# GregoryFaust/yaha

Hardware: AMD Instinct MI355X
Metric: aligned reads/s (whole node), 1 000 bp reads, OQC mode hot path (higher is better)
Workload: dtype int16

## Files before the change

### include/yaha_hip.h

```cpp
#ifndef YAHA_HIP_H
#define YAHA_HIP_H
#include <stdint.h>
#include <stddef.h>
#ifdef __cplusplus
extern "C" {
#endif

#define YGPU_OK            0
#define YGPU_EINVAL      (-1)
#define YGPU_ENODEV      (-2)
#define YGPU_ENOMEM      (-3)
#define YGPU_EOVERFLOW   (-4)
#define YGPU_EINTERNAL   (-5)
#define YGPU_EBUSY       (-6)

typedef struct ygpu_params {
    int32_t wordLen;
    int32_t maxHits;
    int32_t bandWidth;
    int32_t maxGap;
    int32_t maxIntron;
    int32_t minMatch;
    int32_t maxDesert;
    int32_t minNonOverlap;
// ... 181 lines not shown
int  ygpu_junctions_collect(ygpu_ctx *ctx, ygpu_junction *out, uint64_t stats[4]);

int  ygpu_inject_results(ygpu_ctx *ctx, const ygpu_result_batch *r);
int  ygpu_selftest_primitives(ygpu_ctx *ctx, uint32_t n, uint32_t seed, int key_bits);
int  ygpu_trace_volume(ygpu_ctx *ctx, uint64_t out[6]);

typedef uint64_t ygpu_ticket;
int  ygpu_submit(ygpu_ctx *ctx, const ygpu_read_batch *batch, ygpu_ticket *ticket);
int  ygpu_poll(ygpu_ctx *ctx, ygpu_ticket ticket);
int  ygpu_wait(ygpu_ctx *ctx, ygpu_ticket ticket, ygpu_result_batch *out);
int  ygpu_last_timing(ygpu_ctx *ctx, float *total_ms, int *n_stages, const char *const **names, const float **ms);


typedef struct ygpu_fragment {
    uint32_t startRefOff;
    uint16_t startQueryOff, endQueryOff;
    uint16_t refLen;
    uint16_t reserved;
    uint32_t read_strand;
} ygpu_fragment;

int  ygpu_seed_join(ygpu_ctx *ctx, const ygpu_fragment **frags, uint64_t *n_frags);

int  ygpu_chain(ygpu_ctx *ctx, const ygpu_fragment **clump_frags, const uint32_t **clump_frag_start,
                const uint32_t **clump_read_strand, uint64_t *n_clumps);

enum { YGPU_DP_FULL = 0, YGPU_DP_BANDED = 1, YGPU_DP_EXT_FWD = 2, YGPU_DP_EXT_REV = 3 };
typedef struct ygpu_dp_problem {
    uint32_t read;
    uint8_t  strand;
    uint8_t  mode;
    uint16_t qOff;
    uint16_t qLen;
    uint16_t rLen;
    uint32_t rOff;
} ygpu_dp_problem;
typedef struct ygpu_dp_result {
    int32_t  score;
    uint16_t addedQLen, addedRLen;
    uint32_t op_start, n_ops;
} ygpu_dp_result;
int  ygpu_dp_batch(ygpu_ctx *ctx, const ygpu_dp_problem *problems, uint32_t n,
                   const ygpu_dp_result **results, const uint32_t **ops, uint64_t *n_ops);
enum { YGPU_DP_KERNELS_AUTO = 0, YGPU_DP_KERNELS_WAVE = 1, YGPU_DP_KERNELS_LANES = 2, YGPU_DP_KERNELS_LANES_CAREFUL = 3 };
int  ygpu_dp_batch_ex(ygpu_ctx *ctx, const ygpu_dp_problem *problems, uint32_t n, int kernels,
                      const ygpu_dp_result **results, const uint32_t **ops, uint64_t *n_ops);
// ... 50 lines not shown
```

### yaha_amd/__init__.py

```python
import ctypes as C
import os

_HERE = os.path.dirname(os.path.abspath(__file__))
LIB_PATH = os.environ.get("YAHA_HIP_LIB", os.path.join(_HERE, "csrc", "libyaha_hip.so"))
CLI_PATH = os.path.join(_HERE, "csrc", "yaha")


class Params(C.Structure):
    _fields_ = [(n, C.c_int32) for n in (
        "wordLen", "maxHits", "bandWidth", "maxGap", "maxIntron", "minMatch", "maxDesert", "minNonOverlap",
        "minRawScore", "minExtLength", "GOCost", "GECost", "RCost", "MScore", "XCutoff")] + [("minIdentity", C.c_float)]


class IndexView(C.Structure):
    _fields_ = [("bases", C.c_void_p), ("n_base_bytes", C.c_uint64), ("maxROff", C.c_uint32),
                ("startingOffs", C.c_void_p), ("ROA", C.c_void_p), ("totalMatches", C.c_uint32), ("wordLen", C.c_int32)]


class ReadBatch(C.Structure):
    _fields_ = [("n_reads", C.c_uint32), ("codes", C.c_void_p), ("offsets", C.c_void_p)]


class Clump(C.Structure):
    _fields_ = [("sro", C.c_uint32), ("sqo", C.c_uint16), ("eqo", C.c_uint16), ("refLen", C.c_uint16),
# ... 131 lines not shown
    _fields_ = [("n_reads", C.c_uint32), ("clump_start", C.POINTER(C.c_uint32)), ("clumps", C.POINTER(OutClump)), ("ops", C.POINTER(C.c_uint32)),
                ("n_clumps", C.c_uint64), ("n_ops", C.c_uint64), ("counters", Counters)]


class ArenaProfile(C.Structure):
    _fields_ = [("n", C.c_uint32), ("last_clump_slots", C.c_uint32), ("cap", C.c_uint64 * 224), ("trace_ratio", C.c_double), ("ops_ratio", C.c_double), ("last_fall", C.c_int64), ("bases", C.c_uint64)]


DP_FULL, DP_BANDED, DP_EXT_FWD, DP_EXT_REV = 0, 1, 2, 3
DP_KERNELS_AUTO, DP_KERNELS_WAVE, DP_KERNELS_LANES, DP_KERNELS_LANES_CAREFUL = 0, 1, 2, 3

EXPORTS = (
    "ygpu_device_count", "ygpu_init", "ygpu_init_multi", "ygpu_clone", "ygpu_destroy", "ygpu_last_error", "ygpu_memory", "ygpu_park", "ygpu_get_arena_profile", "ygpu_presize", "ygpu_upload", "ygpu_upload_nowait", "ygpu_run", "ygpu_collect", "ygpu_result_size", "ygpu_collect_into", "ygpu_host_alloc", "ygpu_host_free", "ygpu_set_postfilter", "ygpu_postfilter_snapshot", "ygpu_postfilter", "ygpu_postfilter_drop", "ygpu_inject_results", "ygpu_selftest_primitives", "ygpu_trace_volume", "ygpu_filtered_size", "ygpu_collect_filtered", "ygpu_last_timing",
    "ygpu_depth_enable", "ygpu_depth_size", "ygpu_depth_collect", "yaha_session_depth_params",
    "ygpu_events_enable", "ygpu_events_size", "ygpu_events_collect", "yaha_session_events_params",
    "ygpu_pileup_enable", "ygpu_pileup_size", "ygpu_pileup_collect", "ygpu_pileup_candidates_size", "ygpu_pileup_candidates_collect", "ygpu_pileup_gather",
    "yaha_session_pileup_params",
    "ygpu_pileup_add", "ygpu_snv_call_size", "ygpu_snv_collect", "yaha_session_snv_params",
    "ygpu_indels_enable", "ygpu_indels_size", "ygpu_indels_collect", "yaha_session_indel_params",
    "ygpu_eprofile_enable", "ygpu_eprofile_size", "ygpu_eprofile_collect", "yaha_session_eprofile_params",
    "ygpu_junctions_enable", "ygpu_junctions_size", "ygpu_junctions_collect", "yaha_session_junction_params",
    "ygpu_bgzf_open", "ygpu_bgzf_bound", "ygpu_bgzf_compress", "ygpu_bgzf_last_error", "ygpu_bgzf_close",
    "ygpu_bamsort_open", "ygpu_bamsort_append", "ygpu_bamsort_sort", "ygpu_bamsort_next", "ygpu_bamsort_info", "ygpu_bamsort_last_error", "ygpu_bamsort_close",
    "ygpu_submit", "ygpu_poll", "ygpu_wait", "ygpu_seed_join", "ygpu_chain", "ygpu_dp_batch", "ygpu_dp_batch_ex",
    "yaha_session_open", "yaha_session_close", "yaha_session_error", "yaha_session_params",
    "yaha_session_index_view", "yaha_session_header", "yaha_session_next_batch", "yaha_session_emit", "yaha_session_postfilter_params", "yaha_session_emit_filtered",
    "yaha_build_index", "yaha_main")

_lib = None


def lib():
    global _lib
    if _lib is None:
        if not os.path.exists(LIB_PATH):
            raise RuntimeError("%s is missing: run `python -c 'import __graft_entry__ as g; g.build()'` "
                               "(or make -C yaha_amd/csrc); there is no fallback path" % LIB_PATH)
        L = C.CDLL(LIB_PATH)
        L.ygpu_last_error.restype = C.c_char_p
        L.yaha_session_error.restype = C.c_char_p
        L.ygpu_bgzf_last_error.restype = C.c_char_p
        L.ygpu_bgzf_last_error.argtypes = [C.c_void_p]
        L.ygpu_bgzf_bound.restype = C.c_uint64
        L.ygpu_bgzf_bound.argtypes = [C.c_uint64]
        L.ygpu_bamsort_last_error.restype = C.c_char_p
        L.ygpu_bamsort_last_error.argtypes = [C.c_void_p]
        L.ygpu_bamsort_info.restype = C.c_uint64
# ... 264 lines not shown
        nc, no = C.c_uint64(), C.c_uint64()
        self._check(lib().ygpu_filtered_size(self._h, C.byref(nc), C.byref(no)), "ygpu_filtered_size")
        self._f_cs = (C.c_uint32 * (n_reads + 1))(); self._f_cl = (OutClump * max(1, nc.value))(); self._f_ops = (C.c_uint32 * max(1, no.value))()
        r = FilteredBatch()
        self._check(lib().ygpu_collect_filtered(self._h, self._f_cs, self._f_cl, self._f_ops, C.byref(r)), "ygpu_collect_filtered")
        return r

    def trace_volume(self):
        v = (C.c_uint64 * 6)()
        self._check(lib().ygpu_trace_volume(self._h, v), "ygpu_trace_volume")
        return {"records_written": v[0], "records_visitable": v[1], "calls": v[2], "walkers": v[3], "record_bytes": v[4], "arena_bytes": v[5]}

    def timing(self):
        tot, n = C.c_float(), C.c_int()
        names, ms = C.POINTER(C.c_char_p)(), C.POINTER(C.c_float)()
        self._check(lib().ygpu_last_timing(self._h, C.byref(tot), C.byref(n), C.byref(names), C.byref(ms)), "ygpu_last_timing")
        return tot.value, {names[i].decode(): ms[i] for i in range(n.value)}

    def seed_join(self):
        f, n = C.POINTER(Fragment)(), C.c_uint64()
        self._check(lib().ygpu_seed_join(self._h, C.byref(f), C.byref(n)), "ygpu_seed_join")
        return f, n.value

    def chain(self):
        f, s, rs, n = C.POINTER(Fragment)(), C.POINTER(C.c_uint32)(), C.POINTER(C.c_uint32)(), C.c_uint64()
        self._check(lib().ygpu_chain(self._h, C.byref(f), C.byref(s), C.byref(rs), C.byref(n)), "ygpu_chain")
        return f, s, rs, n.value

    def dp_batch(self, problems, kernels=DP_KERNELS_AUTO):
        arr = (DPProblem * len(problems))(*problems)
        res, ops, nops = C.POINTER(DPResult)(), C.POINTER(C.c_uint32)(), C.c_uint64()
        self._check(lib().ygpu_dp_batch_ex(self._h, arr, len(problems), kernels, C.byref(res), C.byref(ops), C.byref(nops)), "ygpu_dp_batch_ex")
        return res, ops, nops.value

    def submit(self, batch):
        t = C.c_uint64()
        self._check(lib().ygpu_submit(self._h, C.byref(batch), C.byref(t)), "ygpu_submit")
        return t.value

    def poll(self, ticket):
        return lib().ygpu_poll(self._h, C.c_uint64(ticket))

    def wait(self, ticket):
        r = ResultBatch()
        self._check(lib().ygpu_wait(self._h, C.c_uint64(ticket), C.byref(r)), "ygpu_wait")
        return r
# ... 136 lines not shown
```

### yaha_amd/csrc/device/ctx.h

```cpp
#pragma once
#include <hip/hip_runtime.h>
#include <string>
#include <vector>
#include <cstring>
#include <cstdio>
#include <cstdlib>
#include <algorithm>
#include <array>
#include <atomic>
#include <chrono>
#include <thread>
#include <mutex>
#include <condition_variable>
#include <memory>
#include "common.h"
#include "../oqc_core.h"

#define HIPCHK(call) do { hipError_t e_ = (call); \
    if (e_ != hipSuccess) { ctx->err = std::string(#call) + ": " + hipGetErrorString(e_); return YGPU_ENODEV; } } while (0)

#define KL(kern, grid, block, shmem, st, ...) do { hipLaunchKernelGGL(kern, grid, block, shmem, st, __VA_ARGS__); hipError_t e_ = hipGetLastError(); \
    if (e_ != hipSuccess) { ctx->err = std::string("launch of " #kern " failed: ") + hipGetErrorString(e_); return YGPU_ENODEV; } } while (0)

#define YD_MAX_CHUNK_EV 16
// ... 9 lines not shown
        if (keep && p && cap) { hipMemcpyAsync(np, p, cap, hipMemcpyDeviceToDevice, st); hipStreamSynchronize(st); }
        if (p) hipFree(p);
        p = np; cap = ncap; return 0;
    }
    void release() { if (p) hipFree(p); p = nullptr; cap = 0; }
    int ensureExact(size_t bytes)
    {
        if (bytes <= cap) return 0;
        release();
        void *np = nullptr;
        if (hipMalloc(&np, bytes) != hipSuccess) return -1;
        p = np; cap = bytes; return 0;
    }
    template <class T> T *as() const { return (T *)p; }
};

enum {
    CNT_NMULTI = 0, CNT_MAXN, CNT_CLUMPS, CNT_CFRAGS, CNT_QCHAIN, CNT_QALIGN, CNT_OUTCLUMPS, CNT_OUTOPS, CNT_QDP, CNT_DPOPS, CNT_NBIG, CNT_QBIG,
    CNT_STATEOPS, CNT_EXTOPS, CNT_QEXT, CNT_SLOW, CNT_NDP, CNT_NDP16, CNT_GAPOPS, CNT_NPEND,
    CNT_NMULTI2 ,
        CNT_NTINY, CNT_NSMALL, CNT_NMID, CNT_NB12, CNT_NB16,
        CNT_NB24,
    CNT_SEGC,
    CNT_NFRAGS = CNT_SEGC + 16,
    CNT_NREG = CNT_NFRAGS + 3,
    CNT_SCANFAIL = CNT_NREG + 2,
    CNT_N = CNT_NREG + 4
};
enum { T_SEED = 0, T_SORT, T_FRAGS, T_CHAIN, T_ALIGN, T_LAYOUT, T_TOP, T_P1 = T_TOP, T_XROWS, T_XTRACE, T_P3, T_XROWS_DEV, T_XROWS_PK, T_N };

extern std::atomic<int> gCtxPerDevice[64];
extern std::mutex gRowsMu[64];
extern hipEvent_t gRowsEv[64][4];
extern bool gRowsEvValid[64][4];
extern unsigned long long gRowsSeq[64];
extern std::atomic<int> gActiveRuns[64];
extern const char *const kStageNames[T_N];

struct PfSide {
    std::string err;
    hipStream_t stream = nullptr;
    uint32_t *pinned = nullptr;
    hipEvent_t evSync = nullptr;
    DevBuf scanState, counters;
    int device = 0;
};

// ... 70 lines not shown
    DevCounters *snapCtr = nullptr;
    DevCounters snapCtrPlain{};
    unsigned long long snapHits = 0, snapFrags = 0, snapRegions = 0;
    DevBuf oqCs, oqCl, oqOpsIn, oqSeeds, oqQlen;
    std::shared_ptr<TrackImage> track[TRACK_KINDS];
    DevBuf puFwd, puReadOff, puTileCnt, puTileStart, puCand, puSlots, puRows;
    uint64_t puNCand = 0; bool puHaveCand = false;
    DevBuf snvOut;
    uint64_t snvN = 0; bool snvHave = false;
    DevBuf idTable, idStats, idSeqStart, idSeqLen, idBinBase, idTileCnt, idTileStart, idOut;
    bool idSet = false, idAuto = false;
    uint64_t idCap = 0, snapBases = 0;
    uint32_t idMinMapq = 0, idMinLen = 1, idNSeqs = 0, idUsed = 0;
    DevBuf epTable, epSeqs;
    bool epSet = false;
    uint32_t epMinMapq = 0, epNSeqs = 0;
    DevBuf jnCnt, jnStart, jnOut, jnStats, jnSeqStart, jnSeqLen;
    bool jnSet = false, jnDone = false, jnHaveTotal = false;
    uint32_t jnMinMapq = 0, jnNSeqs = 0, jnReads = 0, jnTotal = 0;
    uint32_t hOutCounts[2] = {0, 0};
    uint32_t nHits = 0, nFrags = 0, nRegions = 0, nMulti = 0, nTiny = 0, nSmall = 0, nMid = 0, nBig = 0, maxN = 0;
    int sortRankUsed = 0;
    bool sortRankForced = false;
    uint32_t nClumpSlots = 0, nClumps = 0, nClumpFrags = 0, nOut = 0, nOutOps = 0;
    int stageDone = 0;
    std::vector<uint32_t> hClumpStart, hOps, hClumpFragStart, hClumpRS, hDpOps;
    std::vector<ygpu_clump> hClumps;
    std::vector<ygpu_fragment> hFrags, hClumpFrags;
    std::vector<ygpu_dp_result> hDpRes;
    ygpu_counters hCounters{};
    std::thread worker;
    std::mutex aMu;
    std::condition_variable aCv;
    const ygpu_read_batch *aBatch = nullptr;
    uint64_t aTicket = 0;
    int aRc = 0;
    bool aOpen = false, aDone = false, aQuit = false, aWaiting = false;
    ygpu_result_batch aOut{};
    long long lastFall = -1;
    unsigned int hFall = 0;
    uint32_t *pinned = nullptr;
    hipEvent_t evSync = nullptr;
    hipEvent_t ev[T_N][2];
    float ms[T_N] = {0};
    float totalMs = 0;
    const char *names[T_N];
// ... 80 lines not shown
```

### yaha_amd/csrc/device/seed.h

```cpp
#pragma once
#include "common.h"
#include "lookback.h"

__constant__ unsigned char kComp4[16] = {2, 3, 0, 1, 4, 12, 7, 6, 9, 8, 15, 11, 5, 13, 14, 10};

__global__ void k_revcomp(const uint8_t *fwd, uint8_t *rev, const uint32_t *readOff, uint32_t nReads)
{
    const uint32_t r = blockIdx.x; if (r >= nReads) return;
    const uint32_t o = readOff[r], n = readOff[r + 1] - o;
    for (uint32_t k = threadIdx.x; k < n; k += blockDim.x) rev[o + k] = kComp4[fwd[o + n - 1 - k] & 0xF];
}

__global__ void k_pack4(const uint8_t *codes, uint8_t *packed, uint32_t nBytesOut, uint32_t nCodes)
{
    YD_HIGH_PRIO();
    const uint32_t i = blockIdx.x * blockDim.x + threadIdx.x;
    if (i < nBytesOut) packed[i] = (uint8_t)(((codes[2u * i] & 15u) << 4) | (2u * i + 1u < nCodes ? (codes[2u * i + 1u] & 15u) : 15u));
}

#define YD_LOW_BITS (1u << 22)
__global__ void __launch_bounds__(256) k_low_offsets(const uint32_t *SO, uint32_t nKmerSlots , const uint32_t *ROA, uint32_t total, uint32_t *low)
{
    for (uint64_t j = (uint64_t)blockIdx.x * blockDim.x + threadIdx.x; j < total; j += (uint64_t)gridDim.x * blockDim.x) {
        if (ROA[j] >= 32768u) continue;
// ... 43 lines not shown
__global__ void __launch_bounds__(1024) k_sum_parts(const unsigned int *parts, unsigned long long *counter)
{
    YD_HIGH_PRIO();
    __shared__ unsigned long long sSum;
    if (threadIdx.x == 0) sSum = 0;
    __syncthreads();
    unsigned v = (unsigned)waveSumI((int)parts[threadIdx.x]);
    if ((threadIdx.x & 63u) == 0 && v) atomicAdd(&sSum, (unsigned long long)v);
    __syncthreads();
    if (threadIdx.x == 0 && sSum) atomicAdd(counter, sSum);
}

#define YD_EXPAND_HITS 1024
__global__ void k_expand_starts(const uint32_t *hitOff, uint32_t nKmers, uint32_t *blockG0)
{
    YD_HIGH_PRIO();
    const uint32_t g = blockIdx.x * blockDim.x + threadIdx.x;
    if (g >= nKmers) return;
    const uint32_t a = hitOff[g], b = hitOff[g + 1u];
    if (g == 0u) blockG0[(hitOff[nKmers] + (uint32_t)YD_EXPAND_HITS - 1u) / (uint32_t)YD_EXPAND_HITS] = nKmers;
    for (uint32_t blk = (a + (uint32_t)YD_EXPAND_HITS - 1u) / (uint32_t)YD_EXPAND_HITS; (unsigned long long)blk * YD_EXPAND_HITS < b; blk++) blockG0[blk] = g;
}
__global__ void __launch_bounds__(256) k_expand_hits(const uint32_t *ROA, const uint32_t *posS, const uint32_t *hitOff, const uint32_t *posRsI, const uint32_t *blockG0,
    uint32_t nKmers, uint32_t nHits, unsigned long long *keys)
{
    YD_HIGH_PRIO();
    __shared__ uint32_t sOff[YD_EXPAND_HITS + 2], sS[YD_EXPAND_HITS + 2], sRsI[YD_EXPAND_HITS + 2]; __shared__ __attribute__((aligned(16))) uint32_t sK[YD_EXPAND_HITS];
        __shared__ uint32_t sWave[4];
    const uint32_t t0 = blockIdx.x * YD_EXPAND_HITS, tid = threadIdx.x, lane = tid & 63u, w = tid >> 6;
    const uint32_t g0 = blockG0[blockIdx.x], span = min(min(nKmers + 1u - g0, blockG0[blockIdx.x + 1u] + 2u - g0), (uint32_t)YD_EXPAND_HITS + 2u);
    for (uint32_t k = tid; k < span; k += 256u) { sOff[k] = hitOff[g0 + k]; sS[k] = posS[g0 + k]; sRsI[k] = posRsI[g0 + k]; }
    *(uint4 *)&sK[4u * tid] = make_uint4(0u, 0u, 0u, 0u);
    __syncthreads();
    for (uint32_t k = 1u + tid; k + 1u < span; k += 256u) { const uint32_t o = sOff[k]; if (o > t0 && o - t0 < (uint32_t)YD_EXPAND_HITS && sOff[k + 1u] > o) sK[o - t0] = k; }
    __syncthreads();
    {
        const uint4 v = *(const uint4 *)&sK[4u * tid];
        const uint32_t a0 = v.x, a1 = max(a0, v.y), a2 = max(a1, v.z), a3 = max(a2, v.w);
        const uint32_t incl = waveInclMaxU(a3), excl = (uint32_t)laneUp1((int)incl, 0);
        if (lane == 63u) sWave[w] = incl;
        __syncthreads();
        uint32_t carry = excl;
        for (uint32_t k = 0; k < w; k++) carry = max(carry, sWave[k]);
        *(uint4 *)&sK[4u * tid] = make_uint4(max(carry, a0), max(carry, a1), max(carry, a2), max(carry, a3));
    }
    __syncthreads();
    const uint32_t endOff = g0 + span - 1u >= nKmers ? nHits : sOff[span - 1u];
    uint32_t at[4], rsi[4]; bool in[4];
#pragma unroll
// ... 144 lines not shown
```

### yaha_amd/csrc/device/segsort.h

```cpp
#pragma once
#include <hip/hip_runtime.h>
#include <cstdint>
#include "wgsort.h"

#ifndef YD_SORT_TOP
#define YD_SORT_TOP 31
#endif
#define YD_SEGSORT_MAX (512u * YD_SORT_TOP)

template <unsigned BS, unsigned IPT, bool ATOMIC>
__global__ void __launch_bounds__(BS) __attribute__((amdgpu_waves_per_eu(4))) k_seg_sort(const unsigned long long *in, unsigned long long *out, const uint32_t *segB,
                                                                                         const uint32_t *segE, const uint32_t *list, unsigned int *outOfOrder)
{
    YD_HIGH_PRIO();
    using Sort = WgSort<BS, IPT, ATOMIC>;
    __shared__ typename Sort::Storage st;
    const uint32_t seg = list[blockIdx.x];
    const uint32_t b = segB[seg], len = segE[seg] - b;
    const uint32_t rsHi = (uint32_t)__builtin_amdgcn_readfirstlane((int)(uint32_t)(in[b] >> 32)) & 0xFFFF8000u;
    uint32_t dg[IPT], qo[IPT];
    const uint32_t w0 = (threadIdx.x >> 6) * (64u * IPT) + (threadIdx.x & 63u);
#pragma unroll
    for (unsigned k = 0; k < IPT; k++) {
        const uint32_t idx = w0 + k * 64u;
        const unsigned long long key = idx < len ? in[b + idx] : 0ull;
        dg[k] = (uint32_t)(key >> 15); qo[k] = (uint32_t)(key & 0x7FFFull);
    }
    bool bad = false;
    Sort::sort(dg, qo, len, st, [&](uint32_t pos, uint32_t d, uint32_t q) { out[b + pos] = ((unsigned long long)(rsHi | (d >> 17)) << 32) | (unsigned long long)((d << 15) | q); },
        bad);
    if (ATOMIC && bad) atomicOr(outOfOrder, 1u);
}

#define YD_SEG_NCLASS 12
struct SegClassHi { uint32_t hi[YD_SEG_NCLASS]; };
__global__ void __launch_bounds__(256) k_seg_classify(const uint32_t *segB, const uint32_t *segE, uint32_t nSeg, SegClassHi H,
                                                      uint32_t *lists, uint32_t *bigB, uint32_t *bigE, unsigned int *counts)
{
    YD_HIGH_PRIO();
    const uint32_t s = blockIdx.x * blockDim.x + threadIdx.x; const int lane = (int)(threadIdx.x & 63u);
    uint32_t b = 0, e = 0; int cls = -1;
    if (s < nSeg) {
        b = segB[s]; e = segE[s]; const uint32_t len = e - b;
        if (len) { cls = YD_SEG_NCLASS;
#pragma unroll
            for (int c = YD_SEG_NCLASS - 1; c >= 0; c--) if (len <= H.hi[c]) cls = c; }
        if (bigB) { bigB[s] = cls == YD_SEG_NCLASS ? b : 0u; bigE[s] = cls == YD_SEG_NCLASS ? e : 0u; }
    }
#pragma unroll
    for (int c = 0; c <= YD_SEG_NCLASS; c++) {
        const unsigned long long m = __ballot(cls == c);
        if (m == 0ull) continue;
        unsigned base = 0; const int first = __builtin_ctzll(m);
        if (lane == first) base = atomicAdd(&counts[c], (unsigned)__builtin_popcountll(m));
        base = (unsigned)__builtin_amdgcn_readlane((int)base, first);
        if (cls == c) lists[(size_t)c * nSeg + base + (unsigned)__builtin_popcountll(m & ((1ull << lane) - 1ull))] = s;
    }
}

#define YD_SPLIT_NB 16
__global__ void __launch_bounds__(1024) k_seg_split(const unsigned long long *in, unsigned long long *out, const uint32_t *segB, const uint32_t *segE, const uint32_t *bigList,
                                                    int diagBits, uint32_t *subB, uint32_t *subE)
{
    YD_HIGH_PRIO();
    __shared__ uint32_t sCnt[16][YD_SPLIT_NB];
    const uint32_t seg = bigList[blockIdx.x], b = segB[seg], len = segE[seg] - b, t = threadIdx.x, lane = t & 63u, w = t >> 6;
    int lg = 0; while (lg < 4 && ((len + 6143u) / 6144u) > (1u << lg)) lg++;
    const uint32_t nb = 1u << lg; const int sh = diagBits > lg ? diagBits - lg : 0;
    const uint32_t per = ((len + 15u) / 16u + 63u) & ~63u, k0 = min(len, w * per), k1 = min(len, k0 + per);
    if (t < YD_SPLIT_NB * 16u) sCnt[t & 15u][t >> 4] = 0u;
    __syncthreads();
    for (uint32_t k = k0 + lane; k < k1; k += 64u) { const uint32_t d = (uint32_t)(in[b + k] >> 15); atomicAdd(&sCnt[w][min(d >> sh, nb - 1u)], 1u); }
    __syncthreads();
// ... 84 lines not shown
```

### yaha_amd/csrc/device/stage_seed.hip

```cpp
#include "ctx.h"
#include "seed.h"
#include "segsort.h"

uint32_t ydSegSortMax() { return YD_SEGSORT_MAX; }
size_t ydLowTableBytes() { return YD_LOW_BITS / 8; }
int ydLowOffsets(ygpu_ctx *ctx, const ygpu_index_view *ix)
{
    const uint64_t HT = 1ull << (2 * ix->wordLen);
    if (ix->totalMatches)
        KL(k_low_offsets, dim3((unsigned)std::min<uint64_t>(gridFor(ix->totalMatches, 256), (uint64_t)ctx->nCU * 64)), dim3(256), 0, ctx->stream,
           ctx->dSO.as<uint32_t>(), (uint32_t)HT, ctx->dROA.as<uint32_t>(), (uint32_t)ix->totalMatches, ctx->dLow.as<uint32_t>());
    return 0;
}
__global__ void k_touch(unsigned int *p) { if (p && threadIdx.x == 1000) *p = 0; }
int ydFirstLaunch(ygpu_ctx *ctx) { KL(k_touch, dim3(1), dim3(64), 0, ctx->stream, (unsigned int *)nullptr); return 0; }

static std::atomic<int> gSortFell{0}, gSortInject{-1};
static int sortRank(bool *forced = nullptr)
{
    const char *e = getenv("YGPU_SORT_RANK"); const bool b = e && (e[0] == 'b' || e[0] == 'B'), a = e && (e[0] == 'a' || e[0] == 'A');
    if (forced) *forced = a || b;
    return b ? 1 : (a ? 0 : gSortFell.load());
}
int ydSortRank() { return sortRank(); }
// ... 3 lines not shown
    const uint32_t n = ctx->nReads, K = ctx->nKmers; DevBatch B = devBatch(ctx);
    HIPCHK(hipMemsetAsync(ctx->counters.p, 0, 4 * CNT_N, ctx->stream));
    HIPCHK(hipMemsetAsync(ctx->ctr.p, 0, sizeof(DevCounters), ctx->stream));
    HIPCHK(hipMemsetAsync(ctx->errFlag.p, 0, 4, ctx->stream));
    ctx->nHits = ctx->nFrags = ctx->nRegions = ctx->nMulti = ctx->maxN = ctx->nClumps = ctx->nClumpFrags = ctx->nOut = ctx->nOutOps = 0;
    for (int t = 0; t < T_N; t++) { ctx->ms[t] = 0; ctx->evUsed[t] = false; }
    if (K == 0 || n == 0) return 0;
    EV0(T_SEED);
    ENSURE(ctx->posS, 4ull * (K + 1)); ENSURE(ctx->posC, 4ull * (K + 1)); ENSURE(ctx->posRsI, 4ull * (K + 1)); ENSURE(ctx->hitOff, 4ull * (K + 1));
    HIPCHK(hipMemsetAsync(ctx->posC.p, 0, 4ull * (K + 1), ctx->stream));
    ENSURE(ctx->kmerParts, 4096); HIPCHK(hipMemsetAsync(ctx->kmerParts.p, 0, 4096, ctx->stream));
    KL(k_kmer_lookup, dim3(2 * n), dim3(128), 0, ctx->stream, ctx->P, B, ctx->dSO.as<uint32_t>(), ctx->dROA.as<uint32_t>(), ctx->dLow.as<uint32_t>(), ctx->dKmerOff.as<uint32_t>(),
                       ctx->posS.as<uint32_t>(), ctx->posC.as<uint32_t>(), ctx->posRsI.as<uint32_t>(), ctx->kmerParts.as<unsigned int>());
    KL(k_sum_parts, dim3(1), dim3(1024), 0, ctx->stream, ctx->kmerParts.as<unsigned int>(), ctx->ctr.as<DevCounters>()->v + C_KMER);
    int rc = cubScan(ctx, ctx->posC.as<uint32_t>(), ctx->hitOff.as<uint32_t>(), K + 1); if (rc) return rc;
    EV1(T_SEED);
    uint32_t H = 0; rc = fetchU32(ctx, ctx->hitOff.as<uint32_t>() + K, &H); if (rc) return rc;
    ctx->nHits = H;
    if (H == 0) return 0;
    if (H > 0x7FFFFFF0u) { ctx->err = "too many seed hits in one batch; use a smaller batch"; return YGPU_EOVERFLOW; }
    EV0(T_SORT);
    ctx->sortRankUsed = sortRank(&ctx->sortRankForced);
    ENSURE(ctx->keysA, 8ull * H); ENSURE(ctx->keysB, 8ull * H);
    ENSURE(ctx->expandStart, 4ull * (gridFor(H, YD_EXPAND_HITS) + 1));
    KL(k_expand_starts, dim3(gridFor(K, 256)), dim3(256), 0, ctx->stream, ctx->hitOff.as<uint32_t>(), K, ctx->expandStart.as<uint32_t>());
    KL(k_expand_hits, dim3(gridFor(H, YD_EXPAND_HITS)), dim3(256), 0, ctx->stream, ctx->dROA.as<uint32_t>(), ctx->posS.as<uint32_t>(), ctx->hitOff.as<uint32_t>(),
        ctx->posRsI.as<uint32_t>(), ctx->expandStart.as<uint32_t>(), K, H, ctx->keysA.as<unsigned long long>());
    {
        {
            ENSURE(ctx->segOff, 4ull * (2 * n + 2));
            KL(k_seg_offsets, dim3(gridFor(2 * n + 1, 256)), dim3(256), 0, ctx->stream, ctx->dKmerOff.as<uint32_t>(), ctx->hitOff.as<uint32_t>(), 2 * n,
                ctx->segOff.as<uint32_t>());
            {
                const unsigned long long *in = ctx->keysA.as<unsigned long long>(); unsigned long long *out = ctx->keysB.as<unsigned long long>();
                    const uint32_t *so = ctx->segOff.as<uint32_t>();
                ENSURE(ctx->segLists, 4ull * (YD_SEG_NCLASS + 1) * (2 * n + 1));
                uint32_t *segCnt = ctx->counters.as<uint32_t>() + CNT_SEGC;
                const uint32_t mx = ctx->segSortMax;
                static const uint32_t kShape[YD_SEG_NCLASS] = {1024u, 2048u, 3072u, 4096u, 5120u, 6144u, 7168u, 8192u, 10240u, 12288u, 14336u, YD_SEGSORT_MAX};
                SegClassHi HI; for (int c = 0; c < YD_SEG_NCLASS; c++) HI.hi[c] = std::min(mx, kShape[c]);
                auto sortClasses = [&](const unsigned long long *src, unsigned long long *dst, const uint32_t *sB, const uint32_t *sE, uint32_t nSeg, const uint32_t *lists,
                    const uint32_t *nc) -> int {
#define YD_SORT_CLASS(c, BS, IPT) if (nc[c]) { const uint32_t *cl = lists + (size_t)(c) * nSeg; \
                    if (byBallots) KL((k_seg_sort<BS, IPT, false>), dim3(nc[c]), dim3(BS), 0, ctx->stream, src, dst, sB, sE, cl, ooo); \
                    else KL((k_seg_sort<BS, IPT, true>), dim3(nc[c]), dim3(BS), 0, ctx->stream, src, dst, sB, sE, cl, ooo); }
                    const char *ws = getenv("YGPU_SORT_WIDE"); const int wideShapes = ws ? atoi(ws) : 1;
                    const bool byBallots = ctx->sortRankUsed == 1;
                    unsigned int *ooo = ctx->counters.as<unsigned int>() + CNT_NFRAGS + 2;
                    if (wideShapes) { YD_SORT_CLASS(11, 512, YD_SORT_TOP); YD_SORT_CLASS(10, 512, 28); YD_SORT_CLASS(9, 512, 24); YD_SORT_CLASS(8, 512, 20); }
                    else { YD_SORT_CLASS(11, 1024, 16); YD_SORT_CLASS(10, 1024, 14); YD_SORT_CLASS(9, 1024, 12); YD_SORT_CLASS(8, 1024, 10); }
                    YD_SORT_CLASS(7, 512, 16);
                    YD_SORT_CLASS(6, 512, 14); YD_SORT_CLASS(5, 512, 12); YD_SORT_CLASS(4, 512, 10);
                    YD_SORT_CLASS(3, 256, 16); YD_SORT_CLASS(2, 256, 12); YD_SORT_CLASS(1, 128, 16); YD_SORT_CLASS(0, 128, 8);
#undef YD_SORT_CLASS
                    return 0;
                };
                HIPCHK(hipMemsetAsync(segCnt, 0, 4 * (YD_SEG_NCLASS + 1), ctx->stream));
                uint32_t *lists = ctx->segLists.as<uint32_t>();
                KL(k_seg_classify, dim3(gridFor(2 * n, 256)), dim3(256), 0, ctx->stream, so, so + 1, 2 * n, HI, lists, (uint32_t *)nullptr, (uint32_t *)nullptr, segCnt);
                uint32_t nc[YD_SEG_NCLASS + 1] = {0}; rc = fetchU32(ctx, segCnt, nc, YD_SEG_NCLASS + 1); if (rc) return rc;
                rc = sortClasses(in, out, so, so + 1, 2 * n, lists, nc); if (rc) return rc;
                const uint32_t nBig = nc[YD_SEG_NCLASS];
                if (kTrace) { std::vector<uint32_t> so2(2 * (size_t)n + 1); hipMemcpy(so2.data(), so, 4ull * (2 * n + 1), hipMemcpyDeviceToHost);
                    unsigned long long hb = 0, mxl = 0, cl[YD_SEG_NCLASS] = {0};
                    for (uint32_t k = 0; k < 2 * n; k++) { const unsigned long long l = so2[k + 1] - so2[k]; if (l > mx) { hb += l; mxl = std::max(mxl, l);
                        } else for (int c = 0; c < YD_SEG_NCLASS; c++) if (l <= HI.hi[c]) { cl[c] += l; break; } }
                    fprintf(stderr, "[ygpu] hit sort: %u hits; segments above %u hits: %u holding %llu hits (%.1f%%, longest %llu); %% of the hits by class:", H, mx, nBig, hb,
                        100.0 * hb / H, mxl);
                    for (int c = 0; c < YD_SEG_NCLASS; c++) fprintf(stderr, " <=%u: %.1f", HI.hi[c], 100.0 * cl[c] / H);
                    fprintf(stderr, "\n"); }
                if (nBig) {
                    const uint32_t nSub = nBig * YD_SPLIT_NB;
                    ENSURE(ctx->subB, 4ull * nSub + 64); ENSURE(ctx->subE, 4ull * nSub + 64); ENSURE(ctx->subLists, 4ull * (YD_SEG_NCLASS + 1) * nSub + 64);
                    int diagBits = 1; while (diagBits < 32 && (ctx->P.maxROff >> diagBits)) diagBits++;
                    uint32_t *sB = ctx->subB.as<uint32_t>(), *sE = ctx->subE.as<uint32_t>(), *l2 = ctx->subLists.as<uint32_t>();
                    KL(k_seg_split, dim3(nBig), dim3(1024), 0, ctx->stream, in, out, so, so + 1, lists + (size_t)YD_SEG_NCLASS * (2 * n), diagBits, sB, sE);
                    HIPCHK(hipMemsetAsync(segCnt, 0, 4 * (YD_SEG_NCLASS + 1), ctx->stream));
                    KL(k_seg_classify, dim3(gridFor(nSub, 256)), dim3(256), 0, ctx->stream, sB, sE, nSub, HI, l2, (uint32_t *)nullptr, (uint32_t *)nullptr, segCnt);
                    uint32_t ns[YD_SEG_NCLASS + 1] = {0}; rc = fetchU32(ctx, segCnt, ns, YD_SEG_NCLASS + 1); if (rc) return rc;
                    rc = sortClasses(out, out, sB, sE, nSub, l2, ns); if (rc) return rc;
                    uint32_t nOver = ns[YD_SEG_NCLASS]; const uint32_t *oB = sB, *oE = sE, *oList = l2 + (size_t)YD_SEG_NCLASS * nSub;
                    const unsigned long long *cur = out; unsigned long long *other = ctx->keysA.as<unsigned long long>();
                    if (kTrace) { fprintf(stderr, "[ygpu] hit sort: %u long segments cut into buckets, by class:", nBig);
                        for (int c = 0; c < YD_SEG_NCLASS; c++) fprintf(stderr, " %u", ns[c]); fprintf(stderr, "; %u to be cut again\n", nOver); }
                    for (int level = 0; nOver; level++) {
                        if (level >= 12) { ctx->err = "hit sort: a segment does not fit the workgroup sort after twelve cuts"; return YGPU_EINTERNAL; }
                        DevBuf &xB = level & 1 ? ctx->sub3B : ctx->sub2B, &xE = level & 1 ? ctx->sub3E : ctx->sub2E, &xL = level & 1 ? ctx->sub3Lists : ctx->sub2Lists;
                        const uint32_t nSub2 = nOver * YD_SPLIT_NB;
                        ENSURE(xB, 4ull * nSub2 + 64); ENSURE(xE, 4ull * nSub2 + 64); ENSURE(xL, 4ull * (YD_SEG_NCLASS + 1) * nSub2 + 64);
                        KL(k_seg_split_range, dim3(nOver), dim3(1024), 0, ctx->stream, cur, other, out, oB, oE, oList, xB.as<uint32_t>(), xE.as<uint32_t>());
                        HIPCHK(hipMemsetAsync(segCnt, 0, 4 * (YD_SEG_NCLASS + 1), ctx->stream));
                        KL(k_seg_classify, dim3(gridFor(nSub2, 256)), dim3(256), 0, ctx->stream, xB.as<uint32_t>(), xE.as<uint32_t>(), nSub2, HI, xL.as<uint32_t>(),
                            (uint32_t *)nullptr, (uint32_t *)nullptr, segCnt);
                        uint32_t n3[YD_SEG_NCLASS + 1] = {0}; rc = fetchU32(ctx, segCnt, n3, YD_SEG_NCLASS + 1); if (rc) return rc;
                        rc = sortClasses(other, out, xB.as<uint32_t>(), xE.as<uint32_t>(), nSub2, xL.as<uint32_t>(), n3); if (rc) return rc;
                        if (kTrace) fprintf(stderr, "[ygpu] hit sort: cut %d: %u pieces cut again, %u of their buckets still too long\n", level + 2, nOver, n3[YD_SEG_NCLASS]);
                        nOver = n3[YD_SEG_NCLASS]; oB = xB.as<uint32_t>(); oE = xE.as<uint32_t>(); oList = xL.as<uint32_t>() + (size_t)YD_SEG_NCLASS * nSub2;
                        const unsigned long long *was = cur; cur = other; other = (unsigned long long *)was;
                    }
                }
            }
        }
    }
    EV1(T_SORT);
    return 0;
}
template <unsigned BS, unsigned IPT>
static int selftestSegSortShape(ygpu_ctx *ctx, uint64_t &x, char *why, size_t whyLen)
{
    auto rnd = [&]() { x ^= x << 13; x ^= x >> 7; x ^= x << 17; return x; };
    constexpr uint32_t N = BS * IPT; const uint32_t nSeg = 24;
    std::vector<uint32_t> segB(nSeg), segE(nSeg), list(nSeg); std::vector<unsigned long long> keys;
    for (uint32_t sI = 0; sI < nSeg; sI++) {
        const uint32_t pat = sI % 6u;
        uint32_t len = sI == 0 ? 1u : (sI == 1 ? N : (sI == 2 ? N - 63u : (sI == 3 ? 65u : 1u + (uint32_t)(rnd() % N))));
        segB[sI] = (uint32_t)keys.size(); list[sI] = sI;
// ... 124 lines not shown
        HIPCHK(hipMemcpyAsync(ctx->dReadOff.p, ctx->hReadOff.data(), 4ull * (n + 1), hipMemcpyHostToDevice, ctx->stream));
        HIPCHK(hipMemcpyAsync(ctx->dKmerOff.p, ctx->hKmerOff.data(), 4ull * (2 * n + 1), hipMemcpyHostToDevice, ctx->stream));
        KL(k_revcomp, dim3(n), dim3(256), 0, ctx->stream, ctx->dFwd.as<uint8_t>(), ctx->dRev.as<uint8_t>(), ctx->dReadOff.as<uint32_t>(), n);
        const uint32_t nPacked = (uint32_t)((ctx->totalBases + 1) / 2);
        KL(k_pack4, dim3(gridFor(nPacked, 256)), dim3(256), 0, ctx->stream, ctx->dFwd.as<uint8_t>(), ctx->dFwd4.as<uint8_t>(), nPacked, (uint32_t)ctx->totalBases);
        KL(k_pack4, dim3(gridFor(nPacked, 256)), dim3(256), 0, ctx->stream, ctx->dRev.as<uint8_t>(), ctx->dRev4.as<uint8_t>(), nPacked, (uint32_t)ctx->totalBases);
    }
    if (wait) HIPCHK(streamSync(ctx));
    return 0;
}
extern "C" {
int ygpu_upload(ygpu_ctx *ctx, const ygpu_read_batch *b) { return uploadBatch(ctx, b, true); }
int ygpu_upload_nowait(ygpu_ctx *ctx, const ygpu_read_batch *b) { static const bool waitAnyway = getenv("YGPU_UPLOAD_WAIT") != nullptr; return uploadBatch(ctx, b, waitAnyway); }

int ygpu_seed_join(ygpu_ctx *ctx, const ygpu_fragment **frags, uint64_t *n_frags)
{
    if (!ctx || !ctx->stream) return YGPU_EINVAL;
    ctx->stageDone = 0; ctx->keepAllFrags = true; int rc = runTo(ctx, 1); ctx->keepAllFrags = false; if (rc) return rc;
    ctx->hFrags.resize(ctx->nFrags);
    if (ctx->nFrags) HIPCHK(hipMemcpy(ctx->hFrags.data(), ctx->frags.p, 16ull * ctx->nFrags, hipMemcpyDeviceToHost));
    for (auto &f : ctx->hFrags) f.reserved = 0;
    *frags = ctx->hFrags.data(); *n_frags = ctx->nFrags; return 0;
}
}
```

Measured before the change: 444,900.

## Fuse hit expansion into the segmented sort for short seed segments

Adds a fused segmented-sort kernel that builds hit keys straight from ROA, posS and hitOff inside LDS and sorts them, so most segments never write expanded keys to global memory and read them back. The classify pass now runs before expansion and marks which expand blocks are still needed (segments with too many k-mers or too many hits). Only those blocks run in k_expand_hits, and they go through the old sort path. This saves a global write and read of the keys and most expand work, at the cost of a more complex load phase in the sort kernel, lower occupancy hints, and more classification lists. Debug entry points to read segment counts and keys are added as well.

Result: no change. 444,700 (median of 2 runs) (-0.1%).

```diff
diff --git a/include/yaha_hip.h b/include/yaha_hip.h
--- a/include/yaha_hip.h
+++ b/include/yaha_hip.h
@@ -227,6 +227,9 @@
 
 int  ygpu_seed_join(ygpu_ctx *ctx, const ygpu_fragment **frags, uint64_t *n_frags);
 
+int  ygpu_seed_segments(ygpu_ctx *ctx, uint64_t out[4]);
+int  ygpu_seed_keys(ygpu_ctx *ctx, uint64_t *keys, uint64_t cap, uint64_t *n_keys);
+
 int  ygpu_chain(ygpu_ctx *ctx, const ygpu_fragment **clump_frags, const uint32_t **clump_frag_start,
                 const uint32_t **clump_read_strand, uint64_t *n_clumps);
 
diff --git a/yaha_amd/__init__.py b/yaha_amd/__init__.py
--- a/yaha_amd/__init__.py
+++ b/yaha_amd/__init__.py
@@ -177,7 +177,7 @@
     "ygpu_junctions_enable", "ygpu_junctions_size", "ygpu_junctions_collect", "yaha_session_junction_params",
     "ygpu_bgzf_open", "ygpu_bgzf_bound", "ygpu_bgzf_compress", "ygpu_bgzf_last_error", "ygpu_bgzf_close",
     "ygpu_bamsort_open", "ygpu_bamsort_append", "ygpu_bamsort_sort", "ygpu_bamsort_next", "ygpu_bamsort_info", "ygpu_bamsort_last_error", "ygpu_bamsort_close",
-    "ygpu_submit", "ygpu_poll", "ygpu_wait", "ygpu_seed_join", "ygpu_chain", "ygpu_dp_batch", "ygpu_dp_batch_ex",
+    "ygpu_submit", "ygpu_poll", "ygpu_wait", "ygpu_seed_join", "ygpu_seed_segments", "ygpu_seed_keys", "ygpu_chain", "ygpu_dp_batch", "ygpu_dp_batch_ex",
     "yaha_session_open", "yaha_session_close", "yaha_session_error", "yaha_session_params",
     "yaha_session_index_view", "yaha_session_header", "yaha_session_next_batch", "yaha_session_emit", "yaha_session_postfilter_params", "yaha_session_emit_filtered",
     "yaha_build_index", "yaha_main")
@@ -488,6 +488,18 @@
         self._check(lib().ygpu_seed_join(self._h, C.byref(f), C.byref(n)), "ygpu_seed_join")
         return f, n.value
 
+    def seed_segments(self):
+        v = (C.c_uint64 * 4)()
+        self._check(lib().ygpu_seed_segments(self._h, v), "ygpu_seed_segments")
+        return {"fused": v[0], "too_many_kmers": v[1], "long": v[2], "kmer_capacity": v[3]}
+
+    def seed_keys(self):
+        n = C.c_uint64()
+        self._check(lib().ygpu_seed_keys(self._h, None, C.c_uint64(0), C.byref(n)), "ygpu_seed_keys")
+        arr = (C.c_uint64 * max(1, n.value))()
+        self._check(lib().ygpu_seed_keys(self._h, arr, C.c_uint64(n.value), C.byref(n)), "ygpu_seed_keys")
+        return list(arr[:n.value])
+
     def chain(self):
         f, s, rs, n = C.POINTER(Fragment)(), C.POINTER(C.c_uint32)(), C.POINTER(C.c_uint32)(), C.c_uint64()
         self._check(lib().ygpu_chain(self._h, C.byref(f), C.byref(s), C.byref(rs), C.byref(n)), "ygpu_chain")
diff --git a/yaha_amd/csrc/device/ctx.h b/yaha_amd/csrc/device/ctx.h
--- a/yaha_amd/csrc/device/ctx.h
+++ b/yaha_amd/csrc/device/ctx.h
@@ -55,7 +55,7 @@
         CNT_NTINY, CNT_NSMALL, CNT_NMID, CNT_NB12, CNT_NB16,
         CNT_NB24,
     CNT_SEGC,
-    CNT_NFRAGS = CNT_SEGC + 16,
+    CNT_NFRAGS = CNT_SEGC + 32,
     CNT_NREG = CNT_NFRAGS + 3,
     CNT_SCANFAIL = CNT_NREG + 2,
     CNT_N = CNT_NREG + 4
@@ -172,6 +172,7 @@
     uint32_t nHits = 0, nFrags = 0, nRegions = 0, nMulti = 0, nTiny = 0, nSmall = 0, nMid = 0, nBig = 0, maxN = 0;
     int sortRankUsed = 0;
     bool sortRankForced = false;
+    uint32_t seedSegs[3] = {0, 0, 0};
     uint32_t nClumpSlots = 0, nClumps = 0, nClumpFrags = 0, nOut = 0, nOutOps = 0;
     int stageDone = 0;
     std::vector<uint32_t> hClumpStart, hOps, hClumpFragStart, hClumpRS, hDpOps;
diff --git a/yaha_amd/csrc/device/seed.h b/yaha_amd/csrc/device/seed.h
--- a/yaha_amd/csrc/device/seed.h
+++ b/yaha_amd/csrc/device/seed.h
@@ -89,9 +89,10 @@
     for (uint32_t blk = (a + (uint32_t)YD_EXPAND_HITS - 1u) / (uint32_t)YD_EXPAND_HITS; (unsigned long long)blk * YD_EXPAND_HITS < b; blk++) blockG0[blk] = g;
 }
 __global__ void __launch_bounds__(256) k_expand_hits(const uint32_t *ROA, const uint32_t *posS, const uint32_t *hitOff, const uint32_t *posRsI, const uint32_t *blockG0,
-    uint32_t nKmers, uint32_t nHits, unsigned long long *keys)
-{
-    YD_HIGH_PRIO();
+    uint32_t nKmers, uint32_t nHits, unsigned long long *keys, const uint8_t *live)
+{
+    YD_HIGH_PRIO();
+    if (live && !live[blockIdx.x]) return;
     __shared__ uint32_t sOff[YD_EXPAND_HITS + 2], sS[YD_EXPAND_HITS + 2], sRsI[YD_EXPAND_HITS + 2]; __shared__ __attribute__((aligned(16))) uint32_t sK[YD_EXPAND_HITS];
         __shared__ uint32_t sWave[4];
     const uint32_t t0 = blockIdx.x * YD_EXPAND_HITS, tid = threadIdx.x, lane = tid & 63u, w = tid >> 6;
diff --git a/yaha_amd/csrc/device/segsort.h b/yaha_amd/csrc/device/segsort.h
--- a/yaha_amd/csrc/device/segsort.h
+++ b/yaha_amd/csrc/device/segsort.h
@@ -1,6 +1,7 @@
 #pragma once
 #include <hip/hip_runtime.h>
 #include <cstdint>
+#include "seed.h"
 #include "wgsort.h"
 
 #ifndef YD_SORT_TOP
@@ -32,10 +33,75 @@
     if (ATOMIC && bad) atomicOr(outOfOrder, 1u);
 }
 
+#define YD_FUSE_KMERS 2048u
+#define YD_FUSE_KMERS_128 1024u
+#define YD_FUSE_CLASSES_128 2
+template <unsigned BS, unsigned IPT, bool ATOMIC>
+__global__ void __launch_bounds__(BS) __attribute__((amdgpu_waves_per_eu(4))) k_seg_sort_fused(const uint32_t *ROA, const uint32_t *posS, const uint32_t *hitOff,
+    const uint32_t *kmerOff, unsigned long long *out, const uint32_t *list, unsigned int *outOfOrder)
+{
+    YD_HIGH_PRIO();
+    using Sort = WgSort<BS, IPT, ATOMIC>;
+    constexpr unsigned NW = BS / 64u, N = BS * IPT, WN = 64u * IPT;
+    constexpr unsigned KM = BS > 128u ? YD_FUSE_KMERS : YD_FUSE_KMERS_128;
+    struct Load { uint32_t s[KM]; uint16_t o[KM]; uint16_t mark[N]; uint32_t carry[NW]; };
+    union Lds { typename Sort::Storage st; Load ld; };
+    static_assert(sizeof(Load) <= sizeof(typename Sort::Storage), "the load phase lives in the LDS of the passes");
+    __shared__ Lds u;
+    Load &L = u.ld;
+    const uint32_t rs = list[blockIdx.x];
+    const uint32_t g0 = kmerOff[rs], nk = kmerOff[rs + 1u] - g0;
+    const uint32_t b = hitOff[g0], len = hitOff[g0 + nk] - b;
+    const uint32_t tid = threadIdx.x, lane = tid & 63u, w = (uint32_t)__builtin_amdgcn_readfirstlane((int)(tid >> 6));
+    for (uint32_t k = tid; k < nk; k += BS) { L.s[k] = posS[g0 + k]; L.o[k] = (uint16_t)(hitOff[g0 + k] - b); }
+    for (uint32_t e = tid; e < (len + 1u) / 2u; e += BS) ((uint32_t *)L.mark)[e] = 0u;
+    if (tid < NW) L.carry[tid] = 0u;
+    __syncthreads();
+    for (uint32_t k = tid; k < nk; k += BS) {
+        const uint32_t o = L.o[k], oN = k + 1u < nk ? (uint32_t)L.o[k + 1u] : len;
+        if (oN > o) {
+            L.mark[o] = (uint16_t)k;
+            for (uint32_t wb = (o + WN - 1u) / WN; wb * WN < oN; wb++) L.carry[wb] = k;
+        }
+    }
+    __syncthreads();
+    uint32_t dg[IPT], qo[IPT];
+    const uint32_t wbase = w * WN;
+    {
+        uint32_t carry = wbase < len ? L.carry[w] : 0u;
+        carry = (uint32_t)__builtin_amdgcn_readfirstlane((int)carry);
+#pragma unroll
+        for (unsigned k = 0; k < IPT; k++) {
+            const uint32_t row = wbase + k * 64u, idx = row + lane;
+            dg[k] = 0u; qo[k] = 0u;
+            if (row < len) {
+                const uint32_t m = idx < len ? (uint32_t)L.mark[idx] : 0u;
+                const uint32_t km = max(waveInclMaxU(m), carry);
+                carry = (uint32_t)__builtin_amdgcn_readlane((int)km, 63);
+                qo[k] = km; dg[k] = L.s[km] + (idx - (uint32_t)L.o[km]);
+            }
+        }
+    }
+#pragma unroll
+    for (unsigned k = 0; k < IPT; k++) {
+        const bool valid = wbase + k * 64u + lane < len;
+        const uint32_t roff = valid ? ROA[dg[k]] : 0u;
+        dg[k] = valid ? roff - qo[k] : 0u; qo[k] = valid ? qo[k] : 0u;
+    }
+    __syncthreads();
+    const uint32_t rsHi = rs << 15;
+    bool bad = false;
+    Sort::sort(dg, qo, len, u.st, [&](uint32_t pos, uint32_t d,
+        uint32_t q) { out[b + pos] = ((unsigned long long)(rsHi | (d >> 17)) << 32) | (unsigned long long)((d << 15) | q); },
+        bad);
+    if (ATOMIC && bad) atomicOr(outOfOrder, 1u);
+}
+
 #define YD_SEG_NCLASS 12
+#define YD_SEG_NLIST (2 * YD_SEG_NCLASS + 1)
 struct SegClassHi { uint32_t hi[YD_SEG_NCLASS]; };
 __global__ void __launch_bounds__(256) k_seg_classify(const uint32_t *segB, const uint32_t *segE, uint32_t nSeg, SegClassHi H,
-                                                      uint32_t *lists, uint32_t *bigB, uint32_t *bigE, unsigned int *counts)
+                                                      uint32_t *lists, uint32_t *bigB, uint32_t *bigE, unsigned int *counts, const uint32_t *kmerOff, uint8_t *live)
 {
     YD_HIGH_PRIO();
     const uint32_t s = blockIdx.x * blockDim.x + threadIdx.x; const int lane = (int)(threadIdx.x & 63u);
@@ -46,9 +112,13 @@
 #pragma unroll
             for (int c = YD_SEG_NCLASS - 1; c >= 0; c--) if (len <= H.hi[c]) cls = c; }
         if (bigB) { bigB[s] = cls == YD_SEG_NCLASS ? b : 0u; bigE[s] = cls == YD_SEG_NCLASS ? e : 0u; }
-    }
-#pragma unroll
-    for (int c = 0; c <= YD_SEG_NCLASS; c++) {
+        if (kmerOff && cls >= 0) {
+            if (cls < YD_SEG_NCLASS && kmerOff[s + 1u] - kmerOff[s] > (cls < YD_FUSE_CLASSES_128 ? YD_FUSE_KMERS_128 : YD_FUSE_KMERS)) cls += YD_SEG_NCLASS + 1;
+            if (cls >= YD_SEG_NCLASS) for (uint32_t blk = b / (uint32_t)YD_EXPAND_HITS; blk <= (e - 1u) / (uint32_t)YD_EXPAND_HITS; blk++) live[blk] = 1;
+        }
+    }
+    const int nList = kmerOff ? YD_SEG_NLIST : YD_SEG_NCLASS + 1;
+    for (int c = 0; c < nList; c++) {
         const unsigned long long m = __ballot(cls == c);
         if (m == 0ull) continue;
         unsigned base = 0; const int first = __builtin_ctzll(m);
diff --git a/yaha_amd/csrc/device/stage_seed.hip b/yaha_amd/csrc/device/stage_seed.hip
--- a/yaha_amd/csrc/device/stage_seed.hip
+++ b/yaha_amd/csrc/device/stage_seed.hip
@@ -49,10 +49,17 @@
     EV0(T_SORT);
     ctx->sortRankUsed = sortRank(&ctx->sortRankForced);
     ENSURE(ctx->keysA, 8ull * H); ENSURE(ctx->keysB, 8ull * H);
-    ENSURE(ctx->expandStart, 4ull * (gridFor(H, YD_EXPAND_HITS) + 1));
-    KL(k_expand_starts, dim3(gridFor(K, 256)), dim3(256), 0, ctx->stream, ctx->hitOff.as<uint32_t>(), K, ctx->expandStart.as<uint32_t>());
-    KL(k_expand_hits, dim3(gridFor(H, YD_EXPAND_HITS)), dim3(256), 0, ctx->stream, ctx->dROA.as<uint32_t>(), ctx->posS.as<uint32_t>(), ctx->hitOff.as<uint32_t>(),
-        ctx->posRsI.as<uint32_t>(), ctx->expandStart.as<uint32_t>(), K, H, ctx->keysA.as<unsigned long long>());
+    const char *fe = getenv("YGPU_EXPAND_FUSED"); const bool fused = fe ? atoi(fe) != 0 : true;
+    const uint32_t nBlk = (uint32_t)gridFor(H, YD_EXPAND_HITS);
+    ENSURE(ctx->expandStart, 4ull * (nBlk + 1) + nBlk + 64);
+    uint8_t *live = (uint8_t *)(ctx->expandStart.as<uint32_t>() + nBlk + 1);
+    auto expandHits = [&]() -> int {
+        KL(k_expand_starts, dim3(gridFor(K, 256)), dim3(256), 0, ctx->stream, ctx->hitOff.as<uint32_t>(), K, ctx->expandStart.as<uint32_t>());
+        KL(k_expand_hits, dim3(nBlk), dim3(256), 0, ctx->stream, ctx->dROA.as<uint32_t>(), ctx->posS.as<uint32_t>(), ctx->hitOff.as<uint32_t>(),
+            ctx->posRsI.as<uint32_t>(), ctx->expandStart.as<uint32_t>(), K, H, ctx->keysA.as<unsigned long long>(), fused ? (const uint8_t *)live : (const uint8_t *)nullptr);
+        return 0;
+    };
+    if (!fused) { rc = expandHits(); if (rc) return rc; }
     {
         {
             ENSURE(ctx->segOff, 4ull * (2 * n + 2));
@@ -61,15 +68,18 @@
             {
                 const unsigned long long *in = ctx->keysA.as<unsigned long long>(); unsigned long long *out = ctx->keysB.as<unsigned long long>();
                     const uint32_t *so = ctx->segOff.as<uint32_t>();
-                ENSURE(ctx->segLists, 4ull * (YD_SEG_NCLASS + 1) * (2 * n + 1));
+                ENSURE(ctx->segLists, 4ull * YD_SEG_NLIST * (2 * n + 1));
                 uint32_t *segCnt = ctx->counters.as<uint32_t>() + CNT_SEGC;
                 const uint32_t mx = ctx->segSortMax;
                 static const uint32_t kShape[YD_SEG_NCLASS] = {1024u, 2048u, 3072u, 4096u, 5120u, 6144u, 7168u, 8192u, 10240u, 12288u, 14336u, YD_SEGSORT_MAX};
                 SegClassHi HI; for (int c = 0; c < YD_SEG_NCLASS; c++) HI.hi[c] = std::min(mx, kShape[c]);
                 auto sortClasses = [&](const unsigned long long *src, unsigned long long *dst, const uint32_t *sB, const uint32_t *sE, uint32_t nSeg, const uint32_t *lists,
                     const uint32_t *nc) -> int {
+                    const uint32_t *roa = ctx->dROA.as<uint32_t>(), *pS = ctx->posS.as<uint32_t>(), *hO = ctx->hitOff.as<uint32_t>(), *kO = ctx->dKmerOff.as<uint32_t>();
 #define YD_SORT_CLASS(c, BS, IPT) if (nc[c]) { const uint32_t *cl = lists + (size_t)(c) * nSeg; \
-                    if (byBallots) KL((k_seg_sort<BS, IPT, false>), dim3(nc[c]), dim3(BS), 0, ctx->stream, src, dst, sB, sE, cl, ooo); \
+                    if (!src) { if (byBallots) KL((k_seg_sort_fused<BS, IPT, false>), dim3(nc[c]), dim3(BS), 0, ctx->stream, roa, pS, hO, kO, dst, cl, ooo); \
+                        else KL((k_seg_sort_fused<BS, IPT, true>), dim3(nc[c]), dim3(BS), 0, ctx->stream, roa, pS, hO, kO, dst, cl, ooo); } \
+                    else if (byBallots) KL((k_seg_sort<BS, IPT, false>), dim3(nc[c]), dim3(BS), 0, ctx->stream, src, dst, sB, sE, cl, ooo); \
                     else KL((k_seg_sort<BS, IPT, true>), dim3(nc[c]), dim3(BS), 0, ctx->stream, src, dst, sB, sE, cl, ooo); }
                     const char *ws = getenv("YGPU_SORT_WIDE"); const int wideShapes = ws ? atoi(ws) : 1;
                     const bool byBallots = ctx->sortRankUsed == 1;
@@ -82,12 +92,20 @@
 #undef YD_SORT_CLASS
                     return 0;
                 };
-                HIPCHK(hipMemsetAsync(segCnt, 0, 4 * (YD_SEG_NCLASS + 1), ctx->stream));
+                HIPCHK(hipMemsetAsync(segCnt, 0, 4 * YD_SEG_NLIST, ctx->stream));
                 uint32_t *lists = ctx->segLists.as<uint32_t>();
-                KL(k_seg_classify, dim3(gridFor(2 * n, 256)), dim3(256), 0, ctx->stream, so, so + 1, 2 * n, HI, lists, (uint32_t *)nullptr, (uint32_t *)nullptr, segCnt);
-                uint32_t nc[YD_SEG_NCLASS + 1] = {0}; rc = fetchU32(ctx, segCnt, nc, YD_SEG_NCLASS + 1); if (rc) return rc;
-                rc = sortClasses(in, out, so, so + 1, 2 * n, lists, nc); if (rc) return rc;
+                if (fused) HIPCHK(hipMemsetAsync(live, 0, nBlk, ctx->stream));
+                KL(k_seg_classify, dim3(gridFor(2 * n, 256)), dim3(256), 0, ctx->stream, so, so + 1, 2 * n, HI, lists, (uint32_t *)nullptr, (uint32_t *)nullptr, segCnt,
+                    fused ? ctx->dKmerOff.as<uint32_t>() : (const uint32_t *)nullptr, live);
+                if (fused) { rc = expandHits(); if (rc) return rc; }
+                uint32_t nc[YD_SEG_NLIST] = {0}; rc = fetchU32(ctx, segCnt, nc, YD_SEG_NLIST); if (rc) return rc;
+                if (fused) {
+                    rc = sortClasses(nullptr, out, so, so + 1, 2 * n, lists, nc); if (rc) return rc;
+                    rc = sortClasses(in, out, so, so + 1, 2 * n, lists + (size_t)(YD_SEG_NCLASS + 1) * (2 * n), nc + YD_SEG_NCLASS + 1); if (rc) return rc;
+                } else { rc = sortClasses(in, out, so, so + 1, 2 * n, lists, nc); if (rc) return rc; }
                 const uint32_t nBig = nc[YD_SEG_NCLASS];
+                ctx->seedSegs[0] = ctx->seedSegs[1] = 0; ctx->seedSegs[2] = nBig;
+                for (int c = 0; c < YD_SEG_NCLASS; c++) { ctx->seedSegs[fused ? 0 : 1] += nc[c]; ctx->seedSegs[1] += nc[YD_SEG_NCLASS + 1 + c]; }
                 if (kTrace) { std::vector<uint32_t> so2(2 * (size_t)n + 1); hipMemcpy(so2.data(), so, 4ull * (2 * n + 1), hipMemcpyDeviceToHost);
                     unsigned long long hb = 0, mxl = 0, cl[YD_SEG_NCLASS] = {0};
                     for (uint32_t k = 0; k < 2 * n; k++) { const unsigned long long l = so2[k + 1] - so2[k]; if (l > mx) { hb += l; mxl = std::max(mxl, l);
@@ -103,7 +121,8 @@
                     uint32_t *sB = ctx->subB.as<uint32_t>(), *sE = ctx->subE.as<uint32_t>(), *l2 = ctx->subLists.as<uint32_t>();
                     KL(k_seg_split, dim3(nBig), dim3(1024), 0, ctx->stream, in, out, so, so + 1, lists + (size_t)YD_SEG_NCLASS * (2 * n), diagBits, sB, sE);
                     HIPCHK(hipMemsetAsync(segCnt, 0, 4 * (YD_SEG_NCLASS + 1), ctx->stream));
-                    KL(k_seg_classify, dim3(gridFor(nSub, 256)), dim3(256), 0, ctx->stream, sB, sE, nSub, HI, l2, (uint32_t *)nullptr, (uint32_t *)nullptr, segCnt);
+                    KL(k_seg_classify, dim3(gridFor(nSub, 256)), dim3(256), 0, ctx->stream, sB, sE, nSub, HI, l2, (uint32_t *)nullptr, (uint32_t *)nullptr, segCnt,
+                        (const uint32_t *)nullptr, (uint8_t *)nullptr);
                     uint32_t ns[YD_SEG_NCLASS + 1] = {0}; rc = fetchU32(ctx, segCnt, ns, YD_SEG_NCLASS + 1); if (rc) return rc;
                     rc = sortClasses(out, out, sB, sE, nSub, l2, ns); if (rc) return rc;
                     uint32_t nOver = ns[YD_SEG_NCLASS]; const uint32_t *oB = sB, *oE = sE, *oList = l2 + (size_t)YD_SEG_NCLASS * nSub;
@@ -118,7 +137,7 @@
                         KL(k_seg_split_range, dim3(nOver), dim3(1024), 0, ctx->stream, cur, other, out, oB, oE, oList, xB.as<uint32_t>(), xE.as<uint32_t>());
                         HIPCHK(hipMemsetAsync(segCnt, 0, 4 * (YD_SEG_NCLASS + 1), ctx->stream));
                         KL(k_seg_classify, dim3(gridFor(nSub2, 256)), dim3(256), 0, ctx->stream, xB.as<uint32_t>(), xE.as<uint32_t>(), nSub2, HI, xL.as<uint32_t>(),
-                            (uint32_t *)nullptr, (uint32_t *)nullptr, segCnt);
+                            (uint32_t *)nullptr, (uint32_t *)nullptr, segCnt, (const uint32_t *)nullptr, (uint8_t *)nullptr);
                         uint32_t n3[YD_SEG_NCLASS + 1] = {0}; rc = fetchU32(ctx, segCnt, n3, YD_SEG_NCLASS + 1); if (rc) return rc;
                         rc = sortClasses(other, out, xB.as<uint32_t>(), xE.as<uint32_t>(), nSub2, xL.as<uint32_t>(), n3); if (rc) return rc;
                         if (kTrace) fprintf(stderr, "[ygpu] hit sort: cut %d: %u pieces cut again, %u of their buckets still too long\n", level + 2, nOver, n3[YD_SEG_NCLASS]);
@@ -289,4 +308,19 @@
     for (auto &f : ctx->hFrags) f.reserved = 0;
     *frags = ctx->hFrags.data(); *n_frags = ctx->nFrags; return 0;
 }
-}
+int ygpu_seed_segments(ygpu_ctx *ctx, uint64_t out[4])
+{
+    if (!ctx || !ctx->stream || !out) return YGPU_EINVAL;
+    out[0] = ctx->seedSegs[0]; out[1] = ctx->seedSegs[1]; out[2] = ctx->seedSegs[2]; out[3] = YD_FUSE_KMERS; return 0;
+}
+int ygpu_seed_keys(ygpu_ctx *ctx, uint64_t *keys, uint64_t cap, uint64_t *n_keys)
+{
+    if (!ctx || !ctx->stream || !n_keys) return YGPU_EINVAL;
+    *n_keys = ctx->nHits;
+    if (!keys || !ctx->nHits) return 0;
+    if (cap < ctx->nHits) { ctx->err = "ygpu_seed_keys: room for fewer keys than the batch has hits"; return YGPU_EINVAL; }
+    HIPCHK(hipSetDevice(ctx->device)); HIPCHK(streamSync(ctx));
+    HIPCHK(hipMemcpy(keys, ctx->keysB.p, 8ull * ctx->nHits, hipMemcpyDeviceToHost));
+    return 0;
+}
+}
```
